# KarelPeeters/kZero

Measured on AMD Instinct MI355X. Metric: self-play NN evals/sec (node), Chess 20x256 ResNet b=256, 1/2/4/8 GPU, higher is better.
Workload: dtype f16; 1 GPU; chess-20x256 attention head, executor batch 256; engines_per_gpu=1, parallelism=dp1 (no collective)

## Files before the change

kzero_amd/csrc/kz_decode_dev.hpp:

```cpp
#pragma once

struct DecodeDev {
    const int64_t *move_offsets;
    const int32_t *move_indices;
    float *values;
    float *probs;
    int *error_flag;
    int policy_len;
    const uint8_t *sym = nullptr;
    const int32_t *policy_map = nullptr;
    int n_sym = 0;
};

inline DecodeDev decode_dev(const DecodeArgs &a, bool on, int policy_len) {
    return DecodeDev{on ? a.move_offsets : nullptr, a.move_indices, a.values, a.probs, a.error_flag, policy_len, a.sym, a.policy_map, a.n_sym};
}

__device__ __forceinline__ float decode_wave_max_nan(float v) {
#pragma unroll
    for (int off = 32; off > 0; off >>= 1) {
        const float o = __shfl_xor(v, off, 64);
        v = (v != v || o != o) ? NAN : fmaxf(v, o);
    }
    return v;
}

__device__ __forceinline__ void decode_raise(const DecodeDev &d, int board) {
    *reinterpret_cast<volatile int *>(d.error_flag) = 1;
    raise_decode_board(d.error_flag, board);
}

__device__ __forceinline__ float decode_wave_sum(float v) {
#pragma unroll
    for (int off = 32; off > 0; off >>= 1) v += __shfl_xor(v, off, 64);
    return v;
}

template <class LogitAt>
__device__ __forceinline__ void decode_board_wave(const DecodeDev &d, int board, int lane, const float *raw, float *stage,
                                                  int cap, LogitAt logit_at) {
    if (lane == 0) {
        const float s0 = raw[0], s1 = raw[1], s2 = raw[2], s3 = raw[3], s4 = raw[4];
        const float m = fmaxf(s1, fmaxf(s2, s3));
        const float e0 = expf(s1 - m), e1 = expf(s2 - m), e2 = expf(s3 - m), sum = e0 + e1 + e2;
        float *v = d.values + (size_t)board * 5;
        v[0] = tanhf(s0);
        v[1] = e0 / sum;
        v[2] = e1 / sum;
        v[3] = e2 / sum;
        v[4] = s4;
        if (!(sum > 0.0f)) decode_raise(d, board);
    }
    const int64_t lo = d.move_offsets[board];
    const int n = (int)(d.move_offsets[board + 1] - lo);
    const int32_t *pmap = nullptr;
    if (d.sym) {
        const int id = d.sym[board];
        if (id < d.n_sym) pmap = d.policy_map + (size_t)id * d.policy_len;
        else if (lane == 0) decode_raise(d, board);
    }
    if (n <= 0) return;
    auto logit_of = [&](int i) {
        int idx = d.move_indices[lo + i];
        if (d.sym) idx = (pmap && idx >= 0 && idx < d.policy_len) ? pmap[idx] : -1;
        return (idx >= 0 && idx < d.policy_len) ? logit_at(idx) : NAN;
    };
    float mx = -INFINITY;
    for (int i = lane; i < n; i += 64) {
        const float v = logit_of(i);
        if (i < cap) stage[i] = v;
        mx = (mx != mx || v != v) ? NAN : fmaxf(mx, v);
    }
    mx = decode_wave_max_nan(mx);
    float sum = 0.0f;
    for (int i = lane; i < n; i += 64) {
        const float e = expf((i < cap ? stage[i] : logit_of(i)) - mx);
        if (i < cap) stage[i] = e;
        sum += e;
    }
    sum = decode_wave_sum(sum);
    if (lane == 0 && !(sum > 0.0f)) decode_raise(d, board);
    for (int i = lane; i < n; i += 64) d.probs[lo + i] = (i < cap ? stage[i] : expf(logit_of(i) - mx)) / sum;
}
```

kzero_amd/csrc/kz_encode_dev.hpp:

```cpp
#pragma once

__device__ __forceinline__ float encoded_plane(const PackedBoards in, int board, int ch, int square, int hw) {
    float f = 0.0f;
    if (ch < in.n_scalar) {
        f = in.scalars[(size_t)board * in.n_scalar + ch];
    } else if (ch < in.n_scalar + in.n_bool) {
        const uint8_t *bb = in.bits + (size_t)board * in.stride;
        if (in.sym) square = in.square_src[min((int)in.sym[board], in.n_sym - 1) * hw + square];
        const unsigned bit = (unsigned)(ch - in.n_scalar) * hw + square;
        f = (float)((bb[bit >> 3] >> (bit & 7)) & 1);
    }
    return f;
}
```

kzero_amd/csrc/kz_tower.hip:

```cpp
#include <cstdlib>
#include <type_traits>
#include <vector>

#include "kz_kernels.hpp"
#include "kz_launch.hpp"

namespace kz {

typedef _Float16 h16;
typedef h16 h16x8 __attribute__((ext_vector_type(8)));
typedef h16 h16x4 __attribute__((ext_vector_type(4)));
typedef float f32x4 __attribute__((ext_vector_type(4)));

namespace {

#include "kz_decode_dev.hpp"
#include "kz_encode_dev.hpp"

constexpr int C = 256;
constexpr int RS = C * 2 + 16;
constexpr int URS = 3 * C * 2 + 16;
constexpr int KSTEPS = 72;
constexpr int HEAD_KSTEPS = 5 * 8;
constexpr int POLICY = 1880, LOGIT_LD = 96;
constexpr int TOWER_PF_MAX = 8;

struct TowerDev {
    const h16 *x0;
    const uint4 *w_stem, *w_tower;
    const float *bias, *post_scale, *post_shift;
    h16 *y;
    int cin_p, batch, depth;
    PackedBoards in;
    const float *sh_w0, *sh_b0, *sh_w1, *sh_b1, *sh_w2, *sh_b2;
    const int32_t *att_idx;
    float *scalars, *policy;
    int *nonfinite_flag;
    int epoch;
    DecodeDev dec;
};

template <int I, int N, class F>
__device__ __forceinline__ void static_for(F &&f) {
    if constexpr (I < N) {
        f(std::integral_constant<int, I>{});
        static_for<I + 1, N>(f);
    }
}

template <int NB>
struct Layout {
    static constexpr int M = NB * 64;
    static constexpr int MT = M / 16;
    static constexpr bool LINE_TILES = NB == 2;
    static constexpr int BPAD = LINE_TILES ? 128 : 0;
    static constexpr int BOARD = 64 * RS + BPAD;
    static constexpr int TS = LINE_TILES ? 8 * RS : 16 * RS;
    static constexpr int IMG = NB * BOARD;
    static constexpr int X_OFF = 0;
    static constexpr int Y_OFF = IMG;
    static constexpr int Z_OFF = 2 * IMG;
    static_assert(Z_OFF % 256 == 0, "zero rows keep the slot pattern of the image rows");
    static constexpr int S_OFF = Z_OFF + 16 * RS;
    static constexpr int TOWER_BYTES = S_OFF + M * 64;
    static constexpr int U_OFF = Z_OFF;
    static constexpr int ACT_OFF = U_OFF + 16 * URS;
    static constexpr int HID_OFF = ACT_OFF + NB * 256 * 4;
    static constexpr int HEADS_BYTES = HID_OFF + NB * 32 * 4;
    static constexpr int LOG_OFF = Y_OFF;
    static constexpr int BYTES = TOWER_BYTES > HEADS_BYTES ? TOWER_BYTES : HEADS_BYTES;
    static_assert(NB * 64 * LOGIT_LD * 4 <= IMG, "logits fit the Y region");
    static constexpr int row_off(int b, int p) { return b * BOARD + p * RS; }
    static_assert(BYTES <= 160 * 1024, "LDS budget");
};

constexpr int SG_VALU = 0x2, SG_SALU = 0x4, SG_MFMA = 0x8, SG_VMEM_READ = 0x20, SG_DS_READ = 0x100;

template <int NB, bool HEADS, int PF, bool WIDE = false, bool PREV = false>
__global__ __launch_bounds__(256, 1) void kz_tower_resident(TowerDev a) {
    using L = Layout<NB>;
    constexpr int M = L::M, MT = L::MT;
    static_assert(PF <= TOWER_PF_MAX, "the refills past the end of the stream must land in its padding");
    extern __shared__ __attribute__((aligned(16))) unsigned char lds[];

    const int tid = threadIdx.x;
    const int wave = __builtin_amdgcn_readfirstlane(tid >> 6);
    const int lane = tid & 63;
    const int fr = lane & 15, kq = lane >> 4;
    const int board0 = blockIdx.x * NB;
    const int layers = 2 * a.depth;
    const int total_ksteps = layers * KSTEPS + (HEADS ? HEAD_KSTEPS : 0);
    const int bias_rows = layers + (HEADS ? 5 : 0);

    const uint4 *wp = a.w_tower + wave * 256 + lane;
    auto wload_prev = [&](int gk, int nt) __attribute__((always_inline)) { return wp[(size_t)gk * 1024 + nt * 64]; };
    typedef const __attribute__((address_space(1))) unsigned char *gptr;
    gptr wk = (gptr)a.w_tower + wave * 4096;
    const unsigned wlane = lane * 16;
    auto wload = [&](gptr k, int nt) __attribute__((always_inline)) {
        typedef unsigned u32x4 __attribute__((ext_vector_type(4)));
        return __builtin_bit_cast(uint4, *reinterpret_cast<const __attribute__((address_space(1))) u32x4 *>(k + wlane + nt * 1024));
    };
    uint4 wreg[PF][4];
#pragma unroll
    for (int s = 0; s < PF; s++) {
        const int g = s < total_ksteps ? s : total_ksteps - 1;
#pragma unroll
        for (int nt = 0; nt < 4; nt++) wreg[s][nt] = PREV ? wload_prev(g, nt) : wload(wk + s * 16384, nt);
    }
    wk += PF * 16384;
    int g = 0;
    auto ring_take = [&](int stage, h16x8 (&af)[4]) __attribute__((always_inline)) {
#pragma unroll
        for (int nt = 0; nt < 4; nt++) af[nt] = *reinterpret_cast<const h16x8 *>(&wreg[stage][nt]);
#ifndef KZ_TW_NO_WLOAD
        if constexpr (PREV) {
            const int gn = g + PF < total_ksteps ? g + PF : total_ksteps - 1;
#pragma unroll
            for (int nt = 0; nt < 4; nt++) wreg[stage][nt] = wload_prev(gn, nt);
        } else {
#pragma unroll
            for (int nt = 0; nt < 4; nt++) wreg[stage][nt] = wload(wk, nt);
        }
#endif
        wk += 16384;
        if constexpr (!PREV) asm("" : "+s"(wk));
    };

    const int sc = WIDE ? a.cin_p >> 5 : 1;
    const int stem_off = WIDE ? L::Y_OFF : L::S_OFF, srow = 64 * sc, spieces = 4 * sc;
    for (int id = tid; id < 16 * RS / 16; id += 256)
        *reinterpret_cast<uint4 *>(lds + L::Z_OFF + id * 16) = make_uint4(0, 0, 0, 0);
    for (int id = tid; id < M * spieces; id += 256) {
        const int row = WIDE ? id / spieces : id >> 2, c = id - row * spieces;
        const int board = board0 + (row >> 6);
        uint4 v = make_uint4(0, 0, 0, 0);
        if (board < a.batch) {
            if (a.in.bits) {
                h16x8 e;
#pragma unroll
                for (int j = 0; j < 8; j++) e[j] = (h16)encoded_plane(a.in, board, c * 8 + j, row & 63, 64);
                v = *reinterpret_cast<const uint4 *>(&e);
            } else {
                v = *reinterpret_cast<const uint4 *>(a.x0 + ((size_t)board0 * 64 + row) * a.cin_p + c * 8);
            }
        }
        *reinterpret_cast<uint4 *>(lds + stem_off + row * srow + c * 16) = v;
    }
    __syncthreads();

    f32x4 acc[4][MT];
    f32x4 bias_next[4];
    auto fetch_bias = [&](int row) __attribute__((always_inline)) {
        const int l = row <= bias_rows ? row : bias_rows;
#pragma unroll
        for (int nt = 0; nt < 4; nt++)
            bias_next[nt] = *reinterpret_cast<const f32x4 *>(a.bias + l * C + wave * 64 + nt * 16 + kq * 4);
    };
    auto init_acc = [&]() __attribute__((always_inline)) {
#pragma unroll
        for (int nt = 0; nt < 4; nt++)
#pragma unroll
            for (int mt = 0; mt < MT; mt++) acc[nt][mt] = bias_next[nt];
    };
    f32x4 post_s[4], post_t[4];
#pragma unroll
    for (int nt = 0; nt < 4; nt++) {
        post_s[nt] = f32x4{1.f, 1.f, 1.f, 1.f};
        post_t[nt] = f32x4{0.f, 0.f, 0.f, 0.f};
    }

    auto relu4 = [](f32x4 v) {
        typedef int i32x4 __attribute__((ext_vector_type(4)));
        i32x4 b = __builtin_bit_cast(i32x4, v);
#pragma unroll
        for (int j = 0; j < 4; j++) b[j] = b[j] > 0 ? b[j] : 0;
        return __builtin_bit_cast(f32x4, b);
    };
    auto to_h4 = [](f32x4 v) { return h16x4{(h16)v[0], (h16)v[1], (h16)v[2], (h16)v[3]}; };

    const int lane_row = L::LINE_TILES ? (fr >> 3) * L::BOARD + (fr & 7) * RS : fr * RS;
    const int epi_base = lane_row + (wave * 64 + kq * 4) * 2;
    auto epilogue = [&](int dst_off, auto relu, auto residual, auto post) __attribute__((always_inline)) {
#pragma unroll
        for (int nt = 0; nt < 4; nt++) {
            h16x4 rx[MT];
            if constexpr (decltype(residual)::value) {
#pragma unroll
                for (int mt = 0; mt < MT; mt++)
                    rx[mt] = *reinterpret_cast<const h16x4 *>(lds + L::X_OFF + epi_base + mt * L::TS + nt * 32);
            }
#pragma unroll
            for (int mt = 0; mt < MT; mt++) {
                const int off = epi_base + mt * L::TS + nt * 32;
                f32x4 v = acc[nt][mt];
                if constexpr (decltype(relu)::value) v = relu4(v);
                if constexpr (decltype(residual)::value) {
#pragma unroll
                    for (int j = 0; j < 4; j++) v[j] += (float)rx[mt][j];
                }
                if constexpr (decltype(post)::value) v = v * post_s[nt] + post_t[nt];
                *reinterpret_cast<h16x4 *>(lds + dst_off + off) = to_h4(v);
            }
        }
    };
    constexpr std::true_type YES{};
    constexpr std::false_type NO{};

    const bool x_is0 = (lane & 7) == 0, x_is7 = (lane & 7) == 7, yo_is0 = (lane & 8) == 0, yo_is1 = !yo_is0;
    auto tap_ok = [&](int mt, int dy, int dx) __attribute__((always_inline)) {
        const bool kill_x = (dx < 0 && x_is0) || (dx > 0 && x_is7);
        if constexpr (L::LINE_TILES) return !(kill_x || (dy < 0 && mt == 0) || (dy > 0 && mt == MT - 1));
        else return !(kill_x || ((mt & 3) == 0 && dy < 0 && yo_is0) || ((mt & 3) == 3 && dy > 0 && yo_is1));
    };

    fetch_bias(0);
    init_acc();
    fetch_bias(1);
    for (int ks = 0; ks < 9 * sc; ks++) {
        const int tap = WIDE ? ks / sc : ks, chunk = ks - tap * sc;
        const int dy = tap / 3 - 1, dx = tap % 3 - 1;
        h16x8 af[4];
#pragma unroll
        for (int nt = 0; nt < 4; nt++) {
            const uint4 t = a.w_stem[((ks * 4 + wave) * 4 + nt) * 64 + lane];
            af[nt] = *reinterpret_cast<const h16x8 *>(&t);
        }
#pragma unroll
        for (int mt = 0; mt < MT; mt++) {
            const bool ok = tap_ok(mt, dy, dx);
            const int p = L::LINE_TILES ? (fr >> 3) * 64 + mt * 8 + (fr & 7) : mt * 16 + fr;
            const int off = ok ? stem_off + (p + dy * 8 + dx) * srow + chunk * 64 + kq * 16 : L::Z_OFF + kq * 16;
            const h16x8 bf = *reinterpret_cast<const h16x8 *>(lds + off);
#pragma unroll
            for (int nt = 0; nt < 4; nt++)
                acc[nt][mt] = __builtin_amdgcn_mfma_f32_16x16x32_f16(af[nt], bf, acc[nt][mt], 0, 0, 0);
        }
    }
    epilogue(L::X_OFF, NO, NO, NO);
    __syncthreads();

    const int kq_off = 256 * (kq & 1) + 128 * (kq >> 1);
    const int frag_base = lane_row + kq_off;
    auto tap_rows = [&](int dy, int dx, int src_off, int (&T)[MT]) __attribute__((always_inline)) {
        const int shifted = frag_base + src_off + (dy * 8 + dx) * RS;
        const int zrow = L::Z_OFF + ((fr + dy * 8 + dx) & 15) * RS + kq_off;
        const int zrow_odd = L::LINE_TILES ? L::Z_OFF + ((fr + dy * 8 + dx + 8) & 15) * RS + kq_off : zrow;
        if constexpr (PREV) {
#pragma unroll
            for (int mt = 0; mt < MT; mt++) T[mt] = tap_ok(mt, dy, dx) ? shifted + mt * L::TS : ((mt & 1) ? zrow_odd : zrow);
        } else {
            int z0 = zrow, z1 = zrow_odd;
            asm("" : "+v"(z0), "+v"(z1));
            const bool kill_x = ((dx < 0) & x_is0) | ((dx > 0) & x_is7);
#pragma unroll
            for (int mt = 0; mt < MT; mt++) {
                bool kill = kill_x;
                if constexpr (!L::LINE_TILES) kill = kill_x | (((mt & 3) == 0) & (dy < 0) & yo_is0) | (((mt & 3) == 3) & (dy > 0) & yo_is1);
                T[mt] = kill ? ((mt & 1) ? z1 : z0) : shifted + mt * L::TS;
            }
        }
    };

    h16x8 bf[2][MT];
    constexpr auto tile_lo = [](int dy) { return L::LINE_TILES && dy < 0 ? 1 : 0; };
    constexpr auto tile_hi = [](int dy) { return L::LINE_TILES && dy > 0 ? MT - 1 : MT; };

    auto conv_plain = [&](auto ndy_tag, int src_off, int dx_lo, int dx_hi) __attribute__((always_inline)) {
        constexpr int NDY = decltype(ndy_tag)::value, DY0 = NDY == 3 ? -1 : 0;
        int T[NDY][MT], Tn[NDY][MT];
#pragma unroll
        for (int i = 0; i < NDY; i++) tap_rows(DY0 + i, dx_lo, src_off, T[i]);
#pragma unroll
        for (int mt = tile_lo(DY0); mt < tile_hi(DY0); mt++) bf[0][mt] = *reinterpret_cast<const h16x8 *>(lds + T[0][mt]);
#pragma nounroll
        for (int dx = dx_lo; dx < dx_hi; dx++) {
#pragma unroll
            for (int i = 0; i < NDY; i++) tap_rows(DY0 + i, dx + 1 < dx_hi ? dx + 1 : dx, src_off, Tn[i]);
            static_for<0, 8 * NDY>([&](auto s_tag) __attribute__((always_inline)) {
                constexpr int s = decltype(s_tag)::value, ch = s / NDY, i = s % NDY, dy = DY0 + i;
                constexpr int stage = s & (PF - 1), cur = s & 1, nxt = cur ^ 1;
                constexpr int lo = tile_lo(dy), hi = tile_hi(dy), nt_ = hi - lo;
                constexpr int in_ = (i + 1) % NDY, chn = i + 1 < NDY ? ch : ch + 1;
                constexpr int lon = tile_lo(DY0 + in_), hin = tile_hi(DY0 + in_), nr = hin - lon;
#ifndef KZ_TW_NO_DSREAD
#pragma unroll
                for (int mt = 0; mt < MT; mt++) {
                    if (mt >= lon && mt < hin)
                        bf[nxt][mt] = *reinterpret_cast<const h16x8 *>(lds + (chn < 8 ? T[in_][mt] + chn * 16 : Tn[in_][mt]));
                }
#endif
                h16x8 af[4];
                ring_take(stage, af);
// ... 49 lines not shown
#pragma unroll
                for (int mt = 0; mt < MT; mt++)
                    bf[nxt][mt] = *reinterpret_cast<const h16x8 *>(lds + (ch < 7 ? T[mt] + (ch + 1) * 16 : Tn[mt]));
#endif
                static_for<0, 3>([&](auto i_tag) __attribute__((always_inline)) {
                    constexpr int i = decltype(i_tag)::value, dy = i - 1, stage = (ch * 3 + i) & (PF - 1);
                    constexpr int lo = tile_lo(dy), hi = tile_hi(dy), nt_ = hi - lo;
                    h16x8 af[4];
                    ring_take(stage, af);
#pragma unroll
                    for (int nt = 0; nt < 4; nt++)
#pragma unroll
                        for (int mt = 0; mt < MT; mt++)
                            if (mt >= lo && mt < hi)
                                acc[nt][mt] = __builtin_amdgcn_mfma_f32_16x16x32_f16(af[nt], bf[cur][mt + dy], acc[nt][mt], 0, 0, 0);
#pragma unroll
                    for (int j = 0; j < 4; j++) {
                        __builtin_amdgcn_sched_group_barrier(SG_MFMA, 1, 0);
                        __builtin_amdgcn_sched_group_barrier(SG_VMEM_READ, 1, 0);
                    }
                    constexpr int nr = i == 0 ? MT : 0;
#pragma unroll
                    for (int j = 0; j < MT; j++) {
                        if (j < nr) {
                            __builtin_amdgcn_sched_group_barrier(SG_MFMA, 1, 0);
                            __builtin_amdgcn_sched_group_barrier(SG_DS_READ, 1, 0);
                        }
                    }
                    constexpr int n_free = 4 * nt_ - (nr + 4), n_alu = ch == 0 && i == 0 ? n_free : 0;
#pragma unroll
                    for (int j = 0; j < 4 * MT; j++) {
                        if (j < n_alu) {
                            __builtin_amdgcn_sched_group_barrier(SG_MFMA, 1, 0);
                            __builtin_amdgcn_sched_group_barrier(SG_VALU | SG_SALU, 2, 0);
                        }
                    }
                    __builtin_amdgcn_sched_group_barrier(SG_MFMA, n_free - n_alu, 0);
                    __builtin_amdgcn_sched_barrier(0);
                    g++;
                });
            });
#pragma unroll
            for (int mt = 0; mt < MT; mt++) T[mt] = Tn[mt];
        }
    };
    constexpr std::integral_constant<int, 3> THREE_ROWS{};
    constexpr std::integral_constant<int, 1> ONE_ROW{};
    auto conv_3x3 = [&](int src_off) __attribute__((always_inline)) {
        if constexpr (L::LINE_TILES && !PREV) conv_3x3_lines(src_off);
        else conv_plain(THREE_ROWS, src_off, -1, 2);
    };
    auto conv_1x1 = [&](int src_off) __attribute__((always_inline)) { conv_plain(ONE_ROW, src_off, 0, 1); };

    for (int layer = 1; layer <= layers; layer++) {
        const bool is_b = (layer & 1) == 0;
        init_acc();
        fetch_bias(layer + 1);
        if (layer == layers) {
#pragma unroll
            for (int nt = 0; nt < 4; nt++) {
                const int oc = wave * 64 + nt * 16 + kq * 4;
                post_s[nt] = *reinterpret_cast<const f32x4 *>(a.post_scale + oc);
                post_t[nt] = *reinterpret_cast<const f32x4 *>(a.post_shift + oc);
            }
        }
        conv_3x3(is_b ? L::Y_OFF : L::X_OFF);
        if (!is_b) epilogue(L::Y_OFF, YES, NO, NO);
        else if (layer != layers) epilogue(L::X_OFF, YES, YES, NO);
        else epilogue(L::X_OFF, YES, YES, YES);
        __syncthreads();
    }

    if constexpr (!HEADS) {
        for (int id = tid; id < M * 32; id += 256) {
            const int p = id >> 5, c16 = id & 31;
            const int board = board0 + (p >> 6);
            if (board < a.batch) {
                const uint4 v = *reinterpret_cast<const uint4 *>(lds + L::X_OFF + L::row_off(p >> 6, p & 63) + c16 * 16);
                *reinterpret_cast<uint4 *>(a.y + ((size_t)board0 * 64 + p) * C + c16 * 8) = v;
            }
        }
    } else {
        {
            float *act = reinterpret_cast<float *>(lds + L::ACT_OFF);
            for (int o = tid; o < NB * 256; o += 256) {
                const int b = o >> 8, c4 = (o >> 6) & 3, p = o & 63;
                const unsigned char *row = lds + L::X_OFF + L::row_off(b, p);
                const float *w = a.sh_w0 + c4 * C;
                float s = a.sh_b0[c4];
#pragma unroll 4
                for (int i = 0; i < C; i += 8) {
                    const h16x8 xv = *reinterpret_cast<const h16x8 *>(row + i * 2);
                    const f32x4 w0 = *reinterpret_cast<const f32x4 *>(w + i), w1 = *reinterpret_cast<const f32x4 *>(w + i + 4);
#pragma unroll
                    for (int j = 0; j < 4; j++) s += (float)xv[j] * w0[j] + (float)xv[4 + j] * w1[j];
                }
                if (!(fabsf(s) <= 3.0e38f) && a.nonfinite_flag && board0 + b < a.batch) {
                    *reinterpret_cast<volatile int *>(a.nonfinite_flag) = a.epoch;
                    raise_nonfinite_board(a.nonfinite_flag, a.epoch, board0 + b);
                }
                act[o] = fmaxf(s, 0.0f);
            }
        }

        {
            const int tb = L::X_OFF + L::row_off(NB == 2 ? fr >> 3 : 0, 56 + (fr & 7)) + kq_off;
            for (int s = 0; s < 3; s++) {
                f32x4 ua[4];
#pragma unroll
                for (int nt = 0; nt < 4; nt++) ua[nt] = bias_next[nt];
                fetch_bias(layers + 2 + s);
#pragma unroll
                for (int ch = 0; ch < 8; ch++) {
                    const h16x8 bf = *reinterpret_cast<const h16x8 *>(lds + tb + ch * 16);
                    h16x8 af[4];
                    ring_take(ch & (PF - 1), af);
#pragma unroll
                    for (int nt = 0; nt < 4; nt++)
                        ua[nt] = __builtin_amdgcn_mfma_f32_16x16x32_f16(af[nt], bf, ua[nt], 0, 0, 0);
                    g++;
                }
                if (NB == 2 || fr < 8) {
#pragma unroll
                    for (int nt = 0; nt < 4; nt++)
                        *reinterpret_cast<h16x4 *>(lds + L::U_OFF + fr * URS + (256 * s + wave * 64 + nt * 16 + kq * 4) * 2) =
                            to_h4(ua[nt]);
                }
            }
        }

        init_acc();
        fetch_bias(layers + 5);
        conv_1x1(L::X_OFF);
        epilogue(L::Y_OFF, NO, NO, NO);

        init_acc();
        conv_1x1(L::X_OFF);
        __syncthreads();
        epilogue(L::X_OFF, NO, NO, NO);
        __syncthreads();

        {
            const float *act = reinterpret_cast<const float *>(lds + L::ACT_OFF);
            float *hid = reinterpret_cast<float *>(lds + L::HID_OFF);
            if (tid < NB * 128) {
                const int pair = tid >> 2, part = tid & 3, b = pair >> 5, j = pair & 31;
                const float *w = a.sh_w1 + j * 256 + part * 64;
                const float *x = act + b * 256 + part * 64;
                float s = 0.0f;
#pragma unroll 4
                for (int i = 0; i < 64; i += 4) {
                    const f32x4 wv = *reinterpret_cast<const f32x4 *>(w + i), xv = *reinterpret_cast<const f32x4 *>(x + i);
                    s += wv[0] * xv[0] + wv[1] * xv[1] + wv[2] * xv[2] + wv[3] * xv[3];
                }
                s += __shfl_xor(s, 1, 64);
                s += __shfl_xor(s, 2, 64);
                if (part == 0) hid[b * 32 + j] = fmaxf(s + a.sh_b1[j], 0.0f);
            }
        }

        constexpr int IT = NB == 2 ? 2 : 1;
        const int hb = NB == 2 ? wave >> 1 : 0;
        const int it0 = NB == 2 ? (wave & 1) * 2 : wave;
        f32x4 la[IT][6];
        {
            int ja[6], ia[IT];
#pragma unroll
            for (int jt = 0; jt < 4; jt++) ja[jt] = L::X_OFF + L::row_off(hb, jt * 16 + fr) + kq_off;
            ja[4] = L::U_OFF + (hb * 8 + (fr & 7)) * URS + (fr >> 3) * 512 + kq_off;
            ja[5] = L::U_OFF + (hb * 8 + (fr & 7)) * URS + 2 * 512 + kq_off;
#pragma unroll
            for (int ii = 0; ii < IT; ii++) ia[ii] = L::Y_OFF + L::row_off(hb, (it0 + ii) * 16 + fr) + kq_off;
#pragma unroll
            for (int ii = 0; ii < IT; ii++)
#pragma unroll
                for (int jt = 0; jt < 6; jt++) la[ii][jt] = f32x4{0.f, 0.f, 0.f, 0.f};
#pragma unroll
            for (int ch = 0; ch < 8; ch++) {
                h16x8 qa[6], qb[IT];
#pragma unroll
                for (int jt = 0; jt < 6; jt++) qa[jt] = *reinterpret_cast<const h16x8 *>(lds + ja[jt] + ch * 16);
#pragma unroll
                for (int ii = 0; ii < IT; ii++) qb[ii] = *reinterpret_cast<const h16x8 *>(lds + ia[ii] + ch * 16);
#pragma unroll
                for (int ii = 0; ii < IT; ii++)
#pragma unroll
                    for (int jt = 0; jt < 6; jt++)
                        la[ii][jt] = __builtin_amdgcn_mfma_f32_16x16x32_f16(qa[jt], qb[ii], la[ii][jt], 0, 0, 0);
            }
        }
        __syncthreads();
        {
            const float inv = 1.0f / sqrtf((float)C);
#pragma unroll
            for (int ii = 0; ii < IT; ii++)
#pragma unroll
                for (int jt = 0; jt < 6; jt++) {
                    const int i = (it0 + ii) * 16 + fr, j = jt * 16 + kq * 4;
                    *reinterpret_cast<f32x4 *>(lds + L::LOG_OFF + ((hb * 64 + i) * LOGIT_LD + j) * 4) = la[ii][jt] * inv;
                }
        }
        const bool decode = a.dec.move_offsets != nullptr;
        float *raw = reinterpret_cast<float *>(lds + L::ACT_OFF);
        if (tid < NB * 5) {
            const int b = tid / 5, k = tid % 5;
            const float *hid = reinterpret_cast<const float *>(lds + L::HID_OFF) + b * 32;
            float s = a.sh_b2[k];
            for (int i = 0; i < 32; i++) s += a.sh_w2[k * 32 + i] * hid[i];
            if (decode) raw[b * 8 + k] = s;
            else if (board0 + b < a.batch) a.scalars[(size_t)(board0 + b) * 5 + k] = s;
        }
        __syncthreads();
        if (decode) {
            if (wave < NB && board0 + wave < a.batch) {
                const float *lg = reinterpret_cast<const float *>(lds + L::LOG_OFF) + wave * 64 * LOGIT_LD;
                float *stage = reinterpret_cast<float *>(lds + L::X_OFF + L::row_off(wave, 0));
                decode_board_wave(a.dec, board0 + wave, lane, raw + wave * 8, stage, 64 * RS / 4,
                                  [&](int idx) { return lg[a.att_idx[idx]]; });
            }
        } else {
            for (int b = 0; b < NB; b++) {
                if (board0 + b >= a.batch) break;
                const float *lg = reinterpret_cast<const float *>(lds + L::LOG_OFF) + b * 64 * LOGIT_LD;
                float *pol = a.policy + (size_t)(board0 + b) * POLICY;
                for (int k = tid; k < POLICY; k += 256) pol[k] = lg[a.att_idx[k]];
            }
        }
    }
}

#ifndef KZ_PF_NB1
#define KZ_PF_NB1 4
#endif
#ifndef KZ_PF_NB2
#define KZ_PF_NB2 4
#endif
constexpr int PF_NB1 = KZ_PF_NB1, PF_NB2 = KZ_PF_NB2;

void pack_1x1(const float *w, uint16_t *dst) {
    static const int kq_base[4] = {0, 128, 64, 192};
    for (int chunk = 0; chunk < 8; chunk++)
        for (int wave = 0; wave < 4; wave++)
            for (int nt = 0; nt < 4; nt++)
                for (int lane = 0; lane < 64; lane++)
                    for (int j = 0; j < 8; j++) {
                        const int oc = 64 * wave + 16 * nt + (lane & 15);
                        const int ch = 8 * chunk + kq_base[lane >> 4] + j;
                        const _Float16 hv = (_Float16)w[(size_t)oc * 256 + ch];
                        uint16_t bits;
                        __builtin_memcpy(&bits, &hv, 2);
                        dst[((((size_t)chunk * 4 + wave) * 4 + nt) * 64 + lane) * 8 + j] = bits;
                    }
}

}

bool tower_resident_supported(int dtype, int h, int w, int channels, int depth, int c_in) {
    return dtype == 1 && h == 8 && w == 8 && channels == C && depth >= 1 && c_in >= 1 && c_in <= 224;
}

bool tower_heads_supported(int policy_kind, int query_channels, int policy_len, int sh_channels, int sh_size) {
    return policy_kind == 2 && query_channels == C && policy_len == POLICY && sh_channels == 4 && sh_size == 32;
}

size_t tower_packed_weight_elems(int cin_p, int depth) {
    return (size_t)9 * C * cin_p + (size_t)2 * depth * 9 * C * C;
}

size_t tower_heads_weight_elems() { return (size_t)HEAD_KSTEPS * 16 * 1024 / 2; }

size_t tower_weight_pad_elems() { return (size_t)TOWER_PF_MAX * 16 * 1024 / 2; }

void tower_pack_weights(const float *oihw, int cout, int cin, int cin_p, uint16_t *dst, bool tap_major) {
    const int nchunk = cin_p / 32;
    const bool rows_inner = cin_p == 256 && !tap_major;
    static const int kq_base[4] = {0, 128, 64, 192};
    for (int tap = 0; tap < 9; tap++)
        for (int chunk = 0; chunk < nchunk; chunk++) {
            const size_t kstep = rows_inner ? ((size_t)(tap % 3) * 8 + chunk) * 3 + tap / 3 : (size_t)tap * nchunk + chunk;
            for (int wave = 0; wave < 4; wave++)
                for (int nt = 0; nt < 4; nt++)
                    for (int lane = 0; lane < 64; lane++)
                        for (int j = 0; j < 8; j++) {
                            const int oc = 64 * wave + 16 * nt + (lane & 15);
                            const int kq = lane >> 4;
                            const int ch = cin_p == 256 ? 8 * chunk + kq_base[kq] + j : 32 * chunk + 8 * kq + j;
                            float v = 0.0f;
                            if (oc < cout && ch < cin) v = oihw[((size_t)oc * cin + ch) * 9 + tap];
                            const _Float16 hv = (_Float16)v;
                            uint16_t bits;
                            __builtin_memcpy(&bits, &hv, 2);
                            dst[(((kstep * 4 + wave) * 4 + nt) * 64 + lane) * 8 + j] = bits;
                        }
        }
}

void tower_pack_heads(const float *w_bulk , const float *b_bulk, const float *w_under ,
                      const float *b_under, uint16_t *dst, float *bias5) {
    const size_t pass = (size_t)8 * 16 * 1024 / 2;
    std::vector<float> tmp((size_t)256 * 256);
    for (int s = 0; s < 3; s++) {
        for (int q = 0; q < 256; q++) {
            for (int c = 0; c < 256; c++) tmp[(size_t)q * 256 + c] = w_under[(size_t)(3 * q + s) * 256 + c];
            bias5[s * 256 + q] = b_under[3 * q + s];
        }
        pack_1x1(tmp.data(), dst + pass * s);
    }
    pack_1x1(w_bulk, dst + pass * 3);
    pack_1x1(w_bulk + (size_t)256 * 256, dst + pass * 4);
    for (int q = 0; q < 256; q++) {
        bias5[3 * 256 + q] = b_bulk[q];
        bias5[4 * 256 + q] = b_bulk[256 + q];
    }
}

namespace {
template <auto Kernel>
void launch_instance(const TowerDev &d, int grid, int bytes, hipStream_t stream) {
    allow_dynamic_lds<Kernel>(bytes);
    Kernel<<<grid, 256, bytes, stream>>>(d);
}
}

void launch_tower_resident(const TowerArgs &t, hipStream_t stream) {
    TowerDev d{};
    d.x0 = static_cast<const h16 *>(t.x0);
    d.w_stem = static_cast<const uint4 *>(t.w_stem);
    d.w_tower = static_cast<const uint4 *>(t.w_tower);
    d.bias = t.bias;
    d.post_scale = t.post_scale;
    d.post_shift = t.post_shift;
    d.y = static_cast<h16 *>(t.y);
    d.cin_p = t.cin_p;
    d.batch = t.batch;
    d.depth = t.depth;
    d.in = t.in;
    d.sh_w0 = t.sh_w0; d.sh_b0 = t.sh_b0; d.sh_w1 = t.sh_w1; d.sh_b1 = t.sh_b1; d.sh_w2 = t.sh_w2; d.sh_b2 = t.sh_b2;
    d.att_idx = t.att_idx;
    d.scalars = t.scalars;
    d.policy = t.policy;
    d.nonfinite_flag = t.nonfinite_flag;
    d.epoch = t.epoch;
    d.dec = decode_dev(t.decode, t.fused_heads, POLICY);
    const bool heads = t.fused_heads;
#ifdef KZ_EXPERIMENTS
    if (t.prev) {
        const int grid = (t.batch + 1) / 2;
        if (t.cin_p > 32) {
            if (heads) launch_instance<kz_tower_resident<2, true, PF_NB2, true, true>>(d, grid, Layout<2>::BYTES, stream);
            else launch_instance<kz_tower_resident<2, false, PF_NB2, true, true>>(d, grid, Layout<2>::BYTES, stream);
        } else if (t.boards_per_wg == 1) {
            if (heads) launch_instance<kz_tower_resident<1, true, PF_NB1, false, true>>(d, t.batch, Layout<1>::BYTES, stream);
            else launch_instance<kz_tower_resident<1, false, PF_NB1, false, true>>(d, t.batch, Layout<1>::BYTES, stream);
        } else {
            if (heads) launch_instance<kz_tower_resident<2, true, PF_NB2, false, true>>(d, grid, Layout<2>::BYTES, stream);
            else launch_instance<kz_tower_resident<2, false, PF_NB2, false, true>>(d, grid, Layout<2>::BYTES, stream);
        }
        return;
    }
#endif
    if (t.cin_p > 32) {
        const int grid = (t.batch + 1) / 2;
        if (heads) launch_instance<kz_tower_resident<2, true, PF_NB2, true>>(d, grid, Layout<2>::BYTES, stream);
        else launch_instance<kz_tower_resident<2, false, PF_NB2, true>>(d, grid, Layout<2>::BYTES, stream);
    } else if (t.boards_per_wg == 1) {
        if (heads) launch_instance<kz_tower_resident<1, true, PF_NB1>>(d, t.batch, Layout<1>::BYTES, stream);
        else launch_instance<kz_tower_resident<1, false, PF_NB1>>(d, t.batch, Layout<1>::BYTES, stream);
    } else {
        const int grid = (t.batch + 1) / 2;
        if (heads) launch_instance<kz_tower_resident<2, true, PF_NB2>>(d, grid, Layout<2>::BYTES, stream);
        else launch_instance<kz_tower_resident<2, false, PF_NB2>>(d, grid, Layout<2>::BYTES, stream);
    }
}

}
```

Before: 550,800 evals/s.

## Prefetch inputs, stem weights, head weights and decode metadata early in resident tower kernel

Issues global loads for packed input bits, scalars, symmetry ids, stem weights, stem bias, head weights and move offsets at kernel start or ahead of use, then stages them in LDS or registers. The goal is to hide global-memory latency in the encode, stem, value-head and decode phases. The 1x1 head loop now preloads its B fragments and interleaves MFMA with VMEM reads through sched_group_barrier, and decode prefetches the first move indices. It also adds optional timestamp instrumentation and compile-time switches back to the old phases. The cost is higher register pressure and more LDS use, which could hurt scheduling.

```diff
diff --git a/kzero_amd/csrc/kz_decode_dev.hpp b/kzero_amd/csrc/kz_decode_dev.hpp
--- a/kzero_amd/csrc/kz_decode_dev.hpp
+++ b/kzero_amd/csrc/kz_decode_dev.hpp
@@ -36,9 +36,25 @@
     return v;
 }
 
+constexpr int DECODE_PRE = 4;
+struct DecodePrefetch {
+    int64_t lo = 0;
+    int n = 0;
+    int id = 0;
+    int idx[DECODE_PRE] = {};
+};
+
+__device__ __forceinline__ void decode_prefetch_moves(const DecodeDev &d, int lane, DecodePrefetch &p) {
+#pragma unroll
+    for (int k = 0; k < DECODE_PRE; k++) {
+        p.idx[k] = -1;
+        if (lane + 64 * k < p.n) p.idx[k] = d.move_indices[p.lo + lane + 64 * k];
+    }
+}
+
 template <class LogitAt>
 __device__ __forceinline__ void decode_board_wave(const DecodeDev &d, int board, int lane, const float *raw, float *stage,
-                                                  int cap, LogitAt logit_at) {
+                                                  int cap, LogitAt logit_at, bool use_pre, const DecodePrefetch &pre) {
     if (lane == 0) {
         const float s0 = raw[0], s1 = raw[1], s2 = raw[2], s3 = raw[3], s4 = raw[4];
         const float m = fmaxf(s1, fmaxf(s2, s3));
@@ -51,11 +67,11 @@
         v[4] = s4;
         if (!(sum > 0.0f)) decode_raise(d, board);
     }
-    const int64_t lo = d.move_offsets[board];
-    const int n = (int)(d.move_offsets[board + 1] - lo);
+    const int64_t lo = use_pre ? pre.lo : d.move_offsets[board];
+    const int n = use_pre ? pre.n : (int)(d.move_offsets[board + 1] - lo);
     const int32_t *pmap = nullptr;
     if (d.sym) {
-        const int id = d.sym[board];
+        const int id = use_pre ? pre.id : (int)d.sym[board];
         if (id < d.n_sym) pmap = d.policy_map + (size_t)id * d.policy_len;
         else if (lane == 0) decode_raise(d, board);
     }
@@ -66,7 +82,31 @@
         return (idx >= 0 && idx < d.policy_len) ? logit_at(idx) : NAN;
     };
     float mx = -INFINITY;
-    for (int i = lane; i < n; i += 64) {
+    int first = lane;
+    if (use_pre) {
+        float pv[DECODE_PRE];
+#pragma unroll
+        for (int k = 0; k < DECODE_PRE; k++) {
+            int idx = pre.idx[k];
+            bool ok = lane + 64 * k < n && idx >= 0 && idx < d.policy_len;
+            if (d.sym) {
+                if (pmap) idx = pmap[ok ? idx : 0];
+                ok = ok && pmap && idx >= 0 && idx < d.policy_len;
+            }
+            pv[k] = logit_at(ok ? idx : 0);
+            if (!ok) pv[k] = NAN;
+        }
+#pragma unroll
+        for (int k = 0; k < DECODE_PRE; k++) {
+            const int i = lane + 64 * k;
+            if (i < n) {
+                if (i < cap) stage[i] = pv[k];
+                mx = (mx != mx || pv[k] != pv[k]) ? NAN : fmaxf(mx, pv[k]);
+            }
+        }
+        first = lane + 64 * DECODE_PRE;
+    }
+    for (int i = first; i < n; i += 64) {
         const float v = logit_of(i);
         if (i < cap) stage[i] = v;
         mx = (mx != mx || v != v) ? NAN : fmaxf(mx, v);
@@ -82,3 +122,9 @@
     if (lane == 0 && !(sum > 0.0f)) decode_raise(d, board);
     for (int i = lane; i < n; i += 64) d.probs[lo + i] = (i < cap ? stage[i] : expf(logit_of(i) - mx)) / sum;
 }
+
+template <class LogitAt>
+__device__ __forceinline__ void decode_board_wave(const DecodeDev &d, int board, int lane, const float *raw, float *stage,
+                                                  int cap, LogitAt logit_at) {
+    decode_board_wave(d, board, lane, raw, stage, cap, logit_at, false, DecodePrefetch{});
+}
diff --git a/kzero_amd/csrc/kz_encode_dev.hpp b/kzero_amd/csrc/kz_encode_dev.hpp
--- a/kzero_amd/csrc/kz_encode_dev.hpp
+++ b/kzero_amd/csrc/kz_encode_dev.hpp
@@ -1,14 +1,20 @@
 #pragma once
 
-__device__ __forceinline__ float encoded_plane(const PackedBoards in, int board, int ch, int square, int hw) {
+__device__ __forceinline__ float encoded_plane(const float *scalars, const uint8_t *bb, int n_scalar, int n_bool, int ch,
+                                               int square, int hw) {
     float f = 0.0f;
-    if (ch < in.n_scalar) {
-        f = in.scalars[(size_t)board * in.n_scalar + ch];
-    } else if (ch < in.n_scalar + in.n_bool) {
-        const uint8_t *bb = in.bits + (size_t)board * in.stride;
-        if (in.sym) square = in.square_src[min((int)in.sym[board], in.n_sym - 1) * hw + square];
-        const unsigned bit = (unsigned)(ch - in.n_scalar) * hw + square;
+    if (ch < n_scalar) {
+        f = scalars[ch];
+    } else if (ch < n_scalar + n_bool) {
+        const unsigned bit = (unsigned)(ch - n_scalar) * hw + square;
         f = (float)((bb[bit >> 3] >> (bit & 7)) & 1);
     }
     return f;
 }
+
+__device__ __forceinline__ float encoded_plane(const PackedBoards in, int board, int ch, int square, int hw) {
+    if (in.sym && ch >= in.n_scalar && ch < in.n_scalar + in.n_bool)
+        square = in.square_src[min((int)in.sym[board], in.n_sym - 1) * hw + square];
+    return encoded_plane(in.scalars + (size_t)board * in.n_scalar, in.bits + (size_t)board * in.stride, in.n_scalar, in.n_bool,
+                         ch, square, hw);
+}
diff --git a/kzero_amd/csrc/kz_tower.hip b/kzero_amd/csrc/kz_tower.hip
--- a/kzero_amd/csrc/kz_tower.hip
+++ b/kzero_amd/csrc/kz_tower.hip
@@ -1,3 +1,6 @@
+#include <atomic>
+#include <mutex>
+#include <cstdio>
 #include <cstdlib>
 #include <type_traits>
 #include <vector>
@@ -37,6 +40,9 @@
     float *scalars, *policy;
     int *nonfinite_flag;
     int epoch;
+#ifdef KZ_TW_STAMPS
+    int stamp_slot;
+#endif
     DecodeDev dec;
 };
 
@@ -63,23 +69,47 @@
     static_assert(Z_OFF % 256 == 0, "zero rows keep the slot pattern of the image rows");
     static constexpr int S_OFF = Z_OFF + 16 * RS;
     static constexpr int TOWER_BYTES = S_OFF + M * 64;
+    static constexpr int MAX_PLANES = 224;
+    static constexpr int STAGE_OFF = TOWER_BYTES;
+    static constexpr int STAGE_BYTES = NB * MAX_PLANES * 8 + 16 + NB * 16 + NB * 4;
+    static_assert(STAGE_OFF % 16 == 0, "16-byte stores into the staging area");
     static constexpr int U_OFF = Z_OFF;
     static constexpr int ACT_OFF = U_OFF + 16 * URS;
     static constexpr int HID_OFF = ACT_OFF + NB * 256 * 4;
     static constexpr int HEADS_BYTES = HID_OFF + NB * 32 * 4;
     static constexpr int LOG_OFF = Y_OFF;
-    static constexpr int BYTES = TOWER_BYTES > HEADS_BYTES ? TOWER_BYTES : HEADS_BYTES;
+    static constexpr int DEC_OFF = TOWER_BYTES > HEADS_BYTES ? TOWER_BYTES : HEADS_BYTES;
+    static constexpr int BYTES = DEC_OFF + NB * 16 + NB * 4 + (NB & 1) * 4;
     static_assert(NB * 64 * LOGIT_LD * 4 <= IMG, "logits fit the Y region");
     static constexpr int row_off(int b, int p) { return b * BOARD + p * RS; }
+    static_assert(STAGE_OFF + STAGE_BYTES <= DEC_OFF, "the encode's staging area fits what the heads phase needs anyway");
     static_assert(BYTES <= 160 * 1024, "LDS budget");
 };
 
 constexpr int SG_VALU = 0x2, SG_SALU = 0x4, SG_MFMA = 0x8, SG_VMEM_READ = 0x20, SG_DS_READ = 0x100;
 
+#ifndef KZ_TW_OLD_PHASES
+#define KZ_TW_OLD_PHASES 0
+#endif
+#ifdef KZ_TW_STAMPS
+constexpr int TW_STAMP_WGS = 1024, TW_STAMP_SLOTS = 4;
+__device__ unsigned long long kz_tw_stamps[TW_STAMP_SLOTS][TW_STAMP_WGS][6];
+#define KZ_TW_STAMP(i)                                                                              \
+    do {                                                                                            \
+        __builtin_amdgcn_sched_barrier(0);                                                          \
+        if (threadIdx.x == 0 && blockIdx.x < TW_STAMP_WGS) kz_tw_stamps[a.stamp_slot][blockIdx.x][i] = wall_clock64(); \
+        __builtin_amdgcn_sched_barrier(0);                                                          \
+    } while (0)
+#else
+#define KZ_TW_STAMP(i) do {} while (0)
+#endif
 template <int NB, bool HEADS, int PF, bool WIDE = false, bool PREV = false>
 __global__ __launch_bounds__(256, 1) void kz_tower_resident(TowerDev a) {
     using L = Layout<NB>;
     constexpr int M = L::M, MT = L::MT;
+    constexpr bool OLD_ENC = PREV || (KZ_TW_OLD_PHASES & 1), OLD_STEM = PREV || (KZ_TW_OLD_PHASES & 2), OLD_H1 = PREV || (KZ_TW_OLD_PHASES & 4),
+                   OLD_H57 = PREV || (KZ_TW_OLD_PHASES & 8), OLD_DEC = PREV || (KZ_TW_OLD_PHASES & 16);
+    KZ_TW_STAMP(0);
     static_assert(PF <= TOWER_PF_MAX, "the refills past the end of the stream must land in its padding");
     extern __shared__ __attribute__((aligned(16))) unsigned char lds[];
 
@@ -92,6 +122,63 @@
     const int total_ksteps = layers * KSTEPS + (HEADS ? HEAD_KSTEPS : 0);
     const int bias_rows = layers + (HEADS ? 5 : 0);
 
+    const bool fused = !OLD_ENC && a.in.bits != nullptr;
+    const int e_ns = min(a.in.n_scalar, a.cin_p), e_nb = min(a.in.n_bool, a.cin_p - e_ns);
+    const int e_rowb = e_nb * 8, e_brow = (e_rowb + 15) & ~15;
+    const int e_valid = min(NB, a.batch - board0);
+    const int e_sc_off = L::STAGE_OFF, e_bits_off = e_sc_off + ((NB * e_ns * 4 + 15) & ~15), e_sym_off = e_bits_off + NB * e_brow;
+    int e_w = 0;
+    if (fused && e_nb > 0) {
+        const unsigned al = (unsigned)reinterpret_cast<uintptr_t>(a.in.bits) | (unsigned)a.in.stride;
+        e_w = (al & 15) == 0 ? 16 : (al & 3) == 0 ? 4 : 1;
+    }
+    constexpr int E_N1 = WIDE ? 14 : 2, E_N4 = WIDE ? 4 : 1, E_NS = WIDE ? 2 : 1;
+    static_assert(E_N1 * 256 >= NB * (WIDE ? 224 : 32) * 8 && E_N4 * 1024 >= NB * (WIDE ? 224 : 32) * 8 && E_NS * 256 >= NB * (WIDE ? 224 : 32), "every staged unit has a thread");
+    unsigned e_v[WIDE ? 14 : 4] = {};
+    float e_s[E_NS] = {};
+    int e_id = 0;
+    auto e_unit = [&](int idx, int per_board, int &b, int &o) __attribute__((always_inline)) {
+        const int i = idx < e_valid * per_board ? idx : 0;
+        b = NB == 2 && i >= per_board ? 1 : 0;
+        o = i - b * per_board;
+    };
+    if (e_w == 16) {
+        int b, o;
+        e_unit(tid, e_brow >> 4, b, o);
+        const uint4 t = *reinterpret_cast<const uint4 *>(a.in.bits + (size_t)(board0 + b) * a.in.stride + o * 16);
+        e_v[0] = t.x; e_v[1] = t.y; e_v[2] = t.z; e_v[3] = t.w;
+    } else if (e_w == 4) {
+#pragma unroll
+        for (int k = 0; k < E_N4; k++) {
+            int b, o;
+            e_unit(tid + k * 256, e_rowb >> 2, b, o);
+            e_v[k] = *reinterpret_cast<const unsigned *>(a.in.bits + (size_t)(board0 + b) * a.in.stride + o * 4);
+        }
+    } else if (e_w == 1) {
+#pragma unroll
+        for (int k = 0; k < E_N1; k++) {
+            int b, o;
+            e_unit(tid + k * 256, e_rowb, b, o);
+            e_v[k] = a.in.bits[(size_t)(board0 + b) * a.in.stride + o];
+        }
+    }
+    if (fused && e_ns > 0) {
+#pragma unroll
+        for (int k = 0; k < E_NS; k++) {
+            int b, o;
+            e_unit(tid + k * 256, e_ns, b, o);
+            e_s[k] = a.in.scalars[(size_t)(board0 + b) * a.in.n_scalar + o];
+        }
+    }
+    if (fused && a.in.sym && tid < e_valid) e_id = a.in.sym[board0 + tid];
+
+    const bool decode = HEADS && a.dec.move_offsets != nullptr;
+    const bool dec_ahead = !OLD_DEC && decode;
+    long long d_off = 0;
+    int d_id = 0;
+    if (dec_ahead && tid < 2 * e_valid) d_off = a.dec.move_offsets[board0 + (tid >> 1) + (tid & 1)];
+    if (dec_ahead && a.dec.sym && tid < e_valid) d_id = a.dec.sym[board0 + tid];
+
     const uint4 *wp = a.w_tower + wave * 256 + lane;
     auto wload_prev = [&](int gk, int nt) __attribute__((always_inline)) { return wp[(size_t)gk * 1024 + nt * 64]; };
     typedef const __attribute__((address_space(1))) unsigned char *gptr;
@@ -129,14 +216,67 @@
 
     const int sc = WIDE ? a.cin_p >> 5 : 1;
     const int stem_off = WIDE ? L::Y_OFF : L::S_OFF, srow = 64 * sc, spieces = 4 * sc;
+    constexpr int SPF = WIDE ? 4 : 9;
+    const int stem_ksteps = 9 * sc;
+    auto stem_wload = [&](int ks, int nt) __attribute__((always_inline)) { return a.w_stem[((ks * 4 + wave) * 4 + nt) * 64 + lane]; };
+    uint4 wst[SPF][4];
+    if constexpr (!OLD_STEM) {
+#pragma unroll
+        for (int s = 0; s < SPF; s++)
+#pragma unroll
+            for (int nt = 0; nt < 4; nt++) wst[s][nt] = stem_wload(s, nt);
+    }
+    f32x4 bias_stem[4];
+    if constexpr (!OLD_STEM) {
+#pragma unroll
+        for (int nt = 0; nt < 4; nt++) bias_stem[nt] = *reinterpret_cast<const f32x4 *>(a.bias + wave * 64 + nt * 16 + kq * 4);
+    }
     for (int id = tid; id < 16 * RS / 16; id += 256)
         *reinterpret_cast<uint4 *>(lds + L::Z_OFF + id * 16) = make_uint4(0, 0, 0, 0);
+    if (fused) {
+        if (e_w == 16) {
+            if (tid < e_valid * (e_brow >> 4)) *reinterpret_cast<uint4 *>(lds + e_bits_off + tid * 16) = make_uint4(e_v[0], e_v[1], e_v[2], e_v[3]);
+        } else if (e_w == 4) {
+#pragma unroll
+            for (int k = 0; k < E_N4; k++) {
+                const int idx = tid + k * 256, per = e_rowb >> 2, b = NB == 2 && idx >= per ? 1 : 0;
+                if (idx < e_valid * per) *reinterpret_cast<unsigned *>(lds + e_bits_off + b * e_brow + (idx - b * per) * 4) = e_v[k];
+            }
+        } else if (e_w == 1) {
+#pragma unroll
+            for (int k = 0; k < E_N1; k++) {
+                const int idx = tid + k * 256, b = NB == 2 && idx >= e_rowb ? 1 : 0;
+                if (idx < e_valid * e_rowb) lds[e_bits_off + b * e_brow + (idx - b * e_rowb)] = (unsigned char)e_v[k];
+            }
+        }
+#pragma unroll
+        for (int k = 0; k < E_NS; k++) {
+            const int idx = tid + k * 256;
+            if (idx < e_valid * e_ns) *reinterpret_cast<float *>(lds + e_sc_off + idx * 4) = e_s[k];
+        }
+        if (tid < NB) *reinterpret_cast<int *>(lds + e_sym_off + tid * 4) = min(e_id, a.in.n_sym - 1);
+    }
+    if (dec_ahead) {
+        if (tid < 2 * NB) *reinterpret_cast<long long *>(lds + L::DEC_OFF + tid * 8) = d_off;
+        if (tid < NB) *reinterpret_cast<int *>(lds + L::DEC_OFF + NB * 16 + tid * 4) = d_id;
+    }
+    if (fused) __syncthreads();
     for (int id = tid; id < M * spieces; id += 256) {
         const int row = WIDE ? id / spieces : id >> 2, c = id - row * spieces;
         const int board = board0 + (row >> 6);
         uint4 v = make_uint4(0, 0, 0, 0);
         if (board < a.batch) {
-            if (a.in.bits) {
+            if (fused) {
+                const int b = row >> 6;
+                int sq = row & 63;
+                if (a.in.sym) sq = a.in.square_src[*reinterpret_cast<const int *>(lds + e_sym_off + b * 4) * 64 + sq];
+                h16x8 e;
+#pragma unroll
+                for (int j = 0; j < 8; j++)
+                    e[j] = (h16)encoded_plane(reinterpret_cast<const float *>(lds + e_sc_off) + b * e_ns, lds + e_bits_off + b * e_brow,
+                                              a.in.n_scalar, a.in.n_bool, c * 8 + j, sq, 64);
+                v = *reinterpret_cast<const uint4 *>(&e);
+            } else if (a.in.bits) {
                 h16x8 e;
 #pragma unroll
                 for (int j = 0; j < 8; j++) e[j] = (h16)encoded_plane(a.in, board, c * 8 + j, row & 63, 64);
@@ -148,6 +288,7 @@
         *reinterpret_cast<uint4 *>(lds + stem_off + row * srow + c * 16) = v;
     }
     __syncthreads();
+    KZ_TW_STAMP(1);
 
     f32x4 acc[4][MT];
     f32x4 bias_next[4];
@@ -214,18 +355,17 @@
         else return !(kill_x || ((mt & 3) == 0 && dy < 0 && yo_is0) || ((mt & 3) == 3 && dy > 0 && yo_is1));
     };
 
-    fetch_bias(0);
+    if constexpr (OLD_STEM) {
+        fetch_bias(0);
+    } else {
+#pragma unroll
+        for (int nt = 0; nt < 4; nt++) bias_next[nt] = bias_stem[nt];
+    }
     init_acc();
     fetch_bias(1);
-    for (int ks = 0; ks < 9 * sc; ks++) {
+    auto stem_step = [&](int ks, const h16x8 (&af)[4]) __attribute__((always_inline)) {
         const int tap = WIDE ? ks / sc : ks, chunk = ks - tap * sc;
         const int dy = tap / 3 - 1, dx = tap % 3 - 1;
-        h16x8 af[4];
-#pragma unroll
-        for (int nt = 0; nt < 4; nt++) {
-            const uint4 t = a.w_stem[((ks * 4 + wave) * 4 + nt) * 64 + lane];
-            af[nt] = *reinterpret_cast<const h16x8 *>(&t);
-        }
 #pragma unroll
         for (int mt = 0; mt < MT; mt++) {
             const bool ok = tap_ok(mt, dy, dx);
@@ -236,9 +376,45 @@
             for (int nt = 0; nt < 4; nt++)
                 acc[nt][mt] = __builtin_amdgcn_mfma_f32_16x16x32_f16(af[nt], bf, acc[nt][mt], 0, 0, 0);
         }
+    };
+    if constexpr (OLD_STEM) {
+        for (int ks = 0; ks < 9 * sc; ks++) {
+            h16x8 af[4];
+#pragma unroll
+            for (int nt = 0; nt < 4; nt++) {
+                const uint4 t = stem_wload(ks, nt);
+                af[nt] = *reinterpret_cast<const h16x8 *>(&t);
+            }
+            stem_step(ks, af);
+        }
+    } else if constexpr (!WIDE) {
+        static_for<0, 9>([&](auto ks_tag) __attribute__((always_inline)) {
+            constexpr int ks = decltype(ks_tag)::value;
+            h16x8 af[4];
+#pragma unroll
+            for (int nt = 0; nt < 4; nt++) af[nt] = *reinterpret_cast<const h16x8 *>(&wst[ks][nt]);
+            stem_step(ks, af);
+        });
+    } else {
+        for (int ks0 = 0; ks0 < stem_ksteps; ks0 += SPF) {
+            static_for<0, SPF>([&](auto s_tag) __attribute__((always_inline)) {
+                constexpr int s = decltype(s_tag)::value;
+                const int ks = ks0 + s;
+                if (ks < stem_ksteps) {
+                    h16x8 af[4];
+#pragma unroll
+                    for (int nt = 0; nt < 4; nt++) af[nt] = *reinterpret_cast<const h16x8 *>(&wst[s][nt]);
+                    const int kn = ks + SPF < stem_ksteps ? ks + SPF : stem_ksteps - 1;
+#pragma unroll
+                    for (int nt = 0; nt < 4; nt++) wst[s][nt] = stem_wload(kn, nt);
+                    stem_step(ks, af);
+                }
+            });
+        }
     }
     epilogue(L::X_OFF, NO, NO, NO);
     __syncthreads();
+    KZ_TW_STAMP(2);
 
     const int kq_off = 256 * (kq & 1) + 128 * (kq >> 1);
     const int frag_base = lane_row + kq_off;
@@ -394,6 +570,8 @@
     };
     auto conv_1x1 = [&](int src_off) __attribute__((always_inline)) { conv_plain(ONE_ROW, src_off, 0, 1); };
 
+    f32x4 h1_w = f32x4{0.f, 0.f, 0.f, 0.f};
+    float h1_b = 0.0f;
     for (int layer = 1; layer <= layers; layer++) {
         const bool is_b = (layer & 1) == 0;
         init_acc();
@@ -405,6 +583,10 @@
                 post_s[nt] = *reinterpret_cast<const f32x4 *>(a.post_scale + oc);
                 post_t[nt] = *reinterpret_cast<const f32x4 *>(a.post_shift + oc);
             }
+            if constexpr (HEADS && !OLD_H1) {
+                h1_w = *reinterpret_cast<const f32x4 *>(a.sh_w0 + wave * C + lane * 4);
+                h1_b = a.sh_b0[wave];
+            }
         }
         conv_3x3(is_b ? L::Y_OFF : L::X_OFF);
         if (!is_b) epilogue(L::Y_OFF, YES, NO, NO);
@@ -412,6 +594,7 @@
         else epilogue(L::X_OFF, YES, YES, YES);
         __syncthreads();
     }
+    KZ_TW_STAMP(3);
 
     if constexpr (!HEADS) {
         for (int id = tid; id < M * 32; id += 256) {
@@ -423,7 +606,29 @@
             }
         }
     } else {
-        {
+        if constexpr (!OLD_H1) {
+            float *act = reinterpret_cast<float *>(lds + L::ACT_OFF);
+            const int wrow = L::Y_OFF + wave * 128;
+            *reinterpret_cast<f32x4 *>(lds + wrow + (lane >> 3) * RS + (lane & 7) * 16) = h1_w;
+            for (int o = tid; o < NB * 256; o += 256) {
+                const int b = o >> 8, p = o & 63;
+                const unsigned char *row = lds + L::X_OFF + L::row_off(b, p);
+                float s = h1_b;
+#pragma unroll 4
+                for (int i = 0; i < C; i += 8) {
+                    const h16x8 xv = *reinterpret_cast<const h16x8 *>(row + i * 2);
+                    const unsigned char *wq = lds + wrow + (i >> 5) * RS + ((i >> 2) & 7) * 16;
+                    const f32x4 w0 = *reinterpret_cast<const f32x4 *>(wq), w1 = *reinterpret_cast<const f32x4 *>(wq + 16);
+#pragma unroll
+                    for (int j = 0; j < 4; j++) s += (float)xv[j] * w0[j] + (float)xv[4 + j] * w1[j];
+                }
+                if (!(fabsf(s) <= 3.0e38f) && a.nonfinite_flag && board0 + b < a.batch) {
+                    *reinterpret_cast<volatile int *>(a.nonfinite_flag) = a.epoch;
+                    raise_nonfinite_board(a.nonfinite_flag, a.epoch, board0 + b);
+                }
+                act[o] = fmaxf(s, 0.0f);
+            }
+        } else {
             float *act = reinterpret_cast<float *>(lds + L::ACT_OFF);
             for (int o = tid; o < NB * 256; o += 256) {
                 const int b = o >> 8, c4 = (o >> 6) & 3, p = o & 63;
@@ -447,19 +652,27 @@
 
         {
             const int tb = L::X_OFF + L::row_off(NB == 2 ? fr >> 3 : 0, 56 + (fr & 7)) + kq_off;
+            h16x8 ubf[8];
+#pragma unroll
+            for (int ch = 0; ch < 8; ch++) ubf[ch] = *reinterpret_cast<const h16x8 *>(lds + tb + ch * 16);
             for (int s = 0; s < 3; s++) {
                 f32x4 ua[4];
 #pragma unroll
                 for (int nt = 0; nt < 4; nt++) ua[nt] = bias_next[nt];
-                fetch_bias(layers + 2 + s);
 #pragma unroll
                 for (int ch = 0; ch < 8; ch++) {
-                    const h16x8 bf = *reinterpret_cast<const h16x8 *>(lds + tb + ch * 16);
+                    if (ch == 1) fetch_bias(layers + 2 + s);
                     h16x8 af[4];
                     ring_take(ch & (PF - 1), af);
 #pragma unroll
                     for (int nt = 0; nt < 4; nt++)
-                        ua[nt] = __builtin_amdgcn_mfma_f32_16x16x32_f16(af[nt], bf, ua[nt], 0, 0, 0);
+                        ua[nt] = __builtin_amdgcn_mfma_f32_16x16x32_f16(af[nt], ubf[ch], ua[nt], 0, 0, 0);
+#pragma unroll
+                    for (int j = 0; j < 4; j++) {
+                        __builtin_amdgcn_sched_group_barrier(SG_MFMA, 1, 0);
+                        __builtin_amdgcn_sched_group_barrier(SG_VMEM_READ, 1, 0);
+                    }
+                    __builtin_amdgcn_sched_barrier(0);
                     g++;
                 }
                 if (NB == 2 || fr < 8) {
@@ -478,6 +691,16 @@
 
         init_acc();
         conv_1x1(L::X_OFF);
+        f32x4 h5_w[16];
+        float h5_b = 0.0f;
+        if constexpr (!OLD_H57) {
+            if (tid < NB * 128) {
+                const int j = (tid >> 2) & 31, part = tid & 3;
+#pragma unroll
+                for (int i = 0; i < 16; i++) h5_w[i] = *reinterpret_cast<const f32x4 *>(a.sh_w1 + j * 256 + part * 64 + i * 4);
+                h5_b = a.sh_b1[j];
+            }
+        }
         __syncthreads();
         epilogue(L::X_OFF, NO, NO, NO);
         __syncthreads();
@@ -487,20 +710,47 @@
             float *hid = reinterpret_cast<float *>(lds + L::HID_OFF);
             if (tid < NB * 128) {
                 const int pair = tid >> 2, part = tid & 3, b = pair >> 5, j = pair & 31;
-                const float *w = a.sh_w1 + j * 256 + part * 64;
+                [[maybe_unused]] const float *w = a.sh_w1 + j * 256 + part * 64;
                 const float *x = act + b * 256 + part * 64;
                 float s = 0.0f;
+                if constexpr (OLD_H57) {
 #pragma unroll 4
-                for (int i = 0; i < 64; i += 4) {
-                    const f32x4 wv = *reinterpret_cast<const f32x4 *>(w + i), xv = *reinterpret_cast<const f32x4 *>(x + i);
-                    s += wv[0] * xv[0] + wv[1] * xv[1] + wv[2] * xv[2] + wv[3] * xv[3];
+                    for (int i = 0; i < 64; i += 4) {
+                        const f32x4 wv = *reinterpret_cast<const f32x4 *>(w + i), xv = *reinterpret_cast<const f32x4 *>(x + i);
+                        s += wv[0] * xv[0] + wv[1] * xv[1] + wv[2] * xv[2] + wv[3] * xv[3];
+                    }
+                    h5_b = a.sh_b1[j];
+                } else {
+#pragma clang fp contract(off)
+#pragma unroll
+                    for (int i = 0; i < 64; i += 4) {
+                        const f32x4 wv = h5_w[i >> 2], xv = *reinterpret_cast<const f32x4 *>(x + i);
+                        s += wv[0] * xv[0] + wv[1] * xv[1] + wv[2] * xv[2] + wv[3] * xv[3];
+                    }
                 }
                 s += __shfl_xor(s, 1, 64);
                 s += __shfl_xor(s, 2, 64);
-                if (part == 0) hid[b * 32 + j] = fmaxf(s + a.sh_b1[j], 0.0f);
-            }
-        }
-
+                if (part == 0) hid[b * 32 + j] = fmaxf(s + h5_b, 0.0f);
+            }
+        }
+
+        const bool dec_wave = dec_ahead && wave < NB && board0 + wave < a.batch;
+        float h7_w[32], h7_b = 0.0f;
+        if constexpr (!OLD_H57) {
+            if (tid < NB * 5) {
+#pragma unroll
+                for (int i = 0; i < 32; i++) h7_w[i] = a.sh_w2[(tid % 5) * 32 + i];
+                h7_b = a.sh_b2[tid % 5];
+            }
+        }
+        DecodePrefetch dpre;
+        if (dec_wave) {
+            const long long *dq = reinterpret_cast<const long long *>(lds + L::DEC_OFF) + wave * 2;
+            dpre.lo = dq[0];
+            dpre.n = (int)(dq[1] - dq[0]);
+            dpre.id = *reinterpret_cast<const int *>(lds + L::DEC_OFF + NB * 16 + wave * 4);
+            decode_prefetch_moves(a.dec, lane, dpre);
+        }
         constexpr int IT = NB == 2 ? 2 : 1;
         const int hb = NB == 2 ? wave >> 1 : 0;
         const int it0 = NB == 2 ? (wave & 1) * 2 : wave;
@@ -542,23 +792,31 @@
                     *reinterpret_cast<f32x4 *>(lds + L::LOG_OFF + ((hb * 64 + i) * LOGIT_LD + j) * 4) = la[ii][jt] * inv;
                 }
         }
-        const bool decode = a.dec.move_offsets != nullptr;
         float *raw = reinterpret_cast<float *>(lds + L::ACT_OFF);
         if (tid < NB * 5) {
             const int b = tid / 5, k = tid % 5;
             const float *hid = reinterpret_cast<const float *>(lds + L::HID_OFF) + b * 32;
-            float s = a.sh_b2[k];
-            for (int i = 0; i < 32; i++) s += a.sh_w2[k * 32 + i] * hid[i];
+            float s;
+            if constexpr (OLD_H57) {
+                s = a.sh_b2[k];
+                for (int i = 0; i < 32; i++) s += a.sh_w2[k * 32 + i] * hid[i];
+            } else {
+                s = h7_b;
+#pragma unroll
+                for (int i = 0; i < 32; i++) s += h7_w[i] * hid[i];
+            }
             if (decode) raw[b * 8 + k] = s;
             else if (board0 + b < a.batch) a.scalars[(size_t)(board0 + b) * 5 + k] = s;
         }
         __syncthreads();
+        KZ_TW_STAMP(4);
         if (decode) {
             if (wave < NB && board0 + wave < a.batch) {
                 const float *lg = reinterpret_cast<const float *>(lds + L::LOG_OFF) + wave * 64 * LOGIT_LD;
                 float *stage = reinterpret_cast<float *>(lds + L::X_OFF + L::row_off(wave, 0));
+                static_assert(64 * RS / 4 >= DECODE_PRE * 64, "the moves fetched ahead are all staged");
                 decode_board_wave(a.dec, board0 + wave, lane, raw + wave * 8, stage, 64 * RS / 4,
-                                  [&](int idx) { return lg[a.att_idx[idx]]; });
+                                  [&](int idx) { return lg[a.att_idx[idx]]; }, dec_wave, dpre);
             }
         } else {
             for (int b = 0; b < NB; b++) {
@@ -569,6 +827,7 @@
             }
         }
     }
+    KZ_TW_STAMP(5);
 }
 
 #ifndef KZ_PF_NB1
@@ -598,6 +857,7 @@
 }
 
 bool tower_resident_supported(int dtype, int h, int w, int channels, int depth, int c_in) {
+    static_assert(Layout<1>::MAX_PLANES == 224 && Layout<2>::MAX_PLANES == 224, "the staging area holds every supported input");
     return dtype == 1 && h == 8 && w == 8 && channels == C && depth >= 1 && c_in >= 1 && c_in <= 224;
 }
 
@@ -664,8 +924,44 @@
 }
 }
 
+#ifdef KZ_TW_STAMPS
+namespace {
+int stamp_slot_of(hipStream_t stream) {
+    static std::mutex mu;
+    static hipStream_t seen[TW_STAMP_SLOTS];
+    static int n = 0;
+    std::lock_guard<std::mutex> lock(mu);
+    for (int i = 0; i < n; i++)
+        if (seen[i] == stream) return i;
+    if (n < TW_STAMP_SLOTS) seen[n++] = stream;
+    return n - 1;
+}
+void dump_stamps(hipStream_t stream, int slot) {
+    static std::atomic<int> launches{0};
+    const char *file = getenv("KZ_TW_STAMP_FILE");
+    const int at = getenv("KZ_TW_STAMP_LAUNCH") ? atoi(getenv("KZ_TW_STAMP_LAUNCH")) : 200;
+    if (!file || launches++ != at) return;
+    (void)hipStreamSynchronize(stream);
+    std::vector<unsigned long long> host((size_t)TW_STAMP_WGS * 6);
+    (void)hipMemcpyFromSymbol(host.data(), HIP_SYMBOL(kz_tw_stamps), host.size() * 8, (size_t)slot * host.size() * 8);
+    if (FILE *f = fopen(file, "wb")) {
+        fwrite(host.data(), 8, host.size(), f);
+        fclose(f);
+    }
+}
+}
+#endif
+
 void launch_tower_resident(const TowerArgs &t, hipStream_t stream) {
     TowerDev d{};
+#ifdef KZ_TW_STAMPS
+    d.stamp_slot = stamp_slot_of(stream);
+    struct DumpAtExit {
+        hipStream_t stream;
+        int slot;
+        ~DumpAtExit() { dump_stamps(stream, slot); }
+    } dump_at_exit{stream, d.stamp_slot};
+#endif
     d.x0 = static_cast<const h16 *>(t.x0);
     d.w_stem = static_cast<const uint4 *>(t.w_stem);
     d.w_tower = static_cast<const uint4 *>(t.w_tower);
```

New measurement: 550,700 evals/s, median of 3. About the same (-0.0%).
